# Peiyannn/MM-PDE

Measured on AMD Instinct MI355X. Metric: MM-PDE rollout node-updates/sec, cylinder 2521-node mesh, 1/2/4/8 GPUs, higher is better.
Workload: dtype f32 (every GNN GEMM fp32-emulated by the fp16x3 split with fp32 accumulate: edge message_net_2, node update_net_1/_2 and message_net_1 projections, embedding; DMM, ItpNet, res_cut, kNN and heads exact fp32); 1 GPU; cy-mmpde; trajectories_per_gpu=16, global_trajectories=16, nodes_per_trajectory=2521, neighbors=35, parallelism=trajectory-shard x1 (no data-path collective), rollout=autoregressive (pred -> next input), launch=eager, three HIP streams, stream_priorities=False

## Files before the change

include/mmpde_hip.h:

```cpp
#ifndef MMPDE_HIP_H
#define MMPDE_HIP_H

#include <stdint.h>

#ifdef __cplusplus
extern "C" {
#endif

#define MMPDE_OK 0
#define MMPDE_ERR_INVALID_ARG (-1)
#define MMPDE_ERR_UNSUPPORTED (-2)
#define MMPDE_ERR_HIP_BASE (-1000)

#define MMPDE_ACT_NONE 0
#define MMPDE_ACT_TANH 1
#define MMPDE_ACT_RELU 2
#define MMPDE_ACT_ELU 3
#define MMPDE_PAD_ZEROS 0
#define MMPDE_PAD_CIRCULAR 1

typedef void *mmpde_stream_t;

int mmpde_version(void);
const char *mmpde_status_string(int status);
// ... 43 lines not shown
int mmpde_radius_graph_binned(const float *pos, const void *bins, int64_t batches, int64_t n_per,
                              float r, int max_num_neighbors, int32_t *nbr_out, int32_t *degree_out,
                              int64_t *stats, mmpde_stream_t stream);

int mmpde_edge_index_from_nbr(const int32_t *nbr, int64_t n, int k, int64_t *edge_index,
                              mmpde_stream_t stream);


int mmpde_linear_skinny(const float *x, int64_t ldx, int64_t m, int64_t k, const float *w,
                        int64_t ldw, const float *b, int64_t n, int act, float *y,
                        int64_t ldy, mmpde_stream_t stream);
int64_t mmpde_linear_skinny_workspace_bytes(int64_t m, int64_t n, int64_t k);
int mmpde_linear_skinny_ws(const float *x, int64_t ldx, int64_t m, int64_t k, const float *w,
                           int64_t ldw, const float *b, int64_t n, int act, float *y, int64_t ldy,
                           float *workspace, int64_t workspace_bytes, mmpde_stream_t stream);

int mmpde_traj_mse(const float *pred, const float *labels, int64_t batches, int64_t n_per,
                   float *out, mmpde_stream_t stream);

int mmpde_resample_bilinear(const float *x, int64_t planes, int h, int w, int oh, int ow, float *y,
                            mmpde_stream_t stream);

int mmpde_conv2d(const float *x, int64_t batches, int cin, int h, int w, const float *weight,
                 const float *bias, int cout, int ks, int stride, int pad,
                 const float *residual, int act, float *y, mmpde_stream_t stream);
int mmpde_conv2d_ex(const float *x, int64_t batches, int cin, int h, int w, const float *weight,
                    const float *bias, int cout, int ks, int stride, int pad, int pad_mode,
                    const float *residual, int res_after_act, int act, float *y,
                    mmpde_stream_t stream);

// ... 243 lines not shown
                         const mmpde_dmm_array_branch *br, const mmpde_dmm_head *hd,
                         void *workspace, float *mesh_out, mmpde_stream_t stream);

int64_t mmpde_dmm_head_cache_bytes(int64_t n_per, int hidden);
int mmpde_dmm_head_prepare(const float *xi, int64_t n_per, const mmpde_dmm_head *hd,
                           void *workspace, void *cache, mmpde_stream_t stream);
int mmpde_dmm_mesh_graph_cached(const float *u, const float *grid, int64_t batches,
                                int64_t n_per, const int32_t *grid_nbr, int k,
                                const mmpde_dmm_graph_branch *br, const mmpde_dmm_head *hd,
                                const void *head_cache, void *workspace, float *mesh_out,
                                mmpde_stream_t stream);
int mmpde_dmm_mesh_array_cached(const float *u, const float *xi, int64_t batches, int64_t n_per,
                                const mmpde_dmm_array_branch *br, const mmpde_dmm_head *hd,
                                const void *head_cache, void *workspace, float *mesh_out,
                                mmpde_stream_t stream);

typedef struct {
    const void *head_cache;
    const void *hess_cache;
    float *hess_out;
    float *det_out;
    float *detmin_out;
    int32_t *folds_out;
    int32_t *folds_total;
} mmpde_dmm_hess_io;
int64_t mmpde_dmm_hess_cache_bytes(int64_t n_per, int hidden);
int mmpde_dmm_hess_prepare(const float *xi, int64_t n_per, const mmpde_dmm_head *hd,
                           void *workspace, void *hess_cache, mmpde_stream_t stream);
int64_t mmpde_dmm_hess_workspace_bytes(int64_t batches, int64_t n_per, int latent, int hidden);
int mmpde_dmm_mesh_graph_hess(const float *u, const float *grid, int64_t batches, int64_t n_per,
// ... 60 lines not shown
```

mm-pde_amd/csrc/dense.hip:

```cpp
#include "common.hpp"

namespace {

constexpr int kSkW = 8;
constexpr int kSkMaxZ = 16;

template <int kSkW>
__global__ __launch_bounds__(kSkW * 64) void linear_skinny_kernel(const float *__restrict__ x,
                                                                  int64_t ldx, int64_t m, int64_t k,
                                                                  const float *__restrict__ w,
                                                                  int64_t ldw,
                                                                  const float *__restrict__ b,
                                                                  int64_t n, int act,
                                                                  float *__restrict__ y, int64_t ldy,
                                                                  int nchz, float *__restrict__ part,
                                                                  unsigned *__restrict__ tickets) {
    constexpr int C = 64 * kSkW, LD = C + 4;
    __shared__ float sw[16 * LD], sx[16 * LD];
    const int tid = threadIdx.x;
    const int wave = tid >> 6;
    const int lane = tid & 63;
    const int r = lane & 15, g = lane >> 4;
    const int64_t col0 = (int64_t)blockIdx.x * 16, row0 = (int64_t)blockIdx.y * 16;
    const int K = (int)k;
    const int c0 = (int)blockIdx.z * nchz;
    const int nch = min((K + C - 1) / C - c0, nchz);
    float lw[16], lx[16];
    auto load = [&](int kc) {
        const int kk = kc + tid;
        const bool ok = kk < K;
        const int o = ok ? kk : 0;
#pragma unroll
        for (int i = 0; i < 16; ++i) {
            const float a = w[min(col0 + i, n - 1) * ldw + o];
            const float c = x[min(row0 + i, m - 1) * ldx + o];
            lw[i] = ok ? a : 0.0f;
            lx[i] = ok ? c : 0.0f;
        }
    };
    f32x4 acc = {0.0f, 0.0f, 0.0f, 0.0f};
    if (nch > 0) load(c0 * C);
    for (int c = 0; c < nch; ++c) {
        if (c) __syncthreads();
#pragma unroll
        for (int i = 0; i < 16; ++i) {
            sw[i * LD + tid] = lw[i];
            sx[i * LD + tid] = lx[i];
        }
        __syncthreads();
        if (c + 1 < nch) load((c0 + c + 1) * C);
        const float *aw = sw + r * LD + 64 * wave + 4 * g;
        const float *ax = sx + r * LD + 64 * wave + 4 * g;
#pragma unroll
        for (int q = 0; q < 4; ++q) {
            const float4 wv = *(const float4 *)(aw + 16 * q);
            const float4 xv = *(const float4 *)(ax + 16 * q);
            acc = mfma16(xv.x, wv.x, acc);
            acc = mfma16(xv.y, wv.y, acc);
            acc = mfma16(xv.z, wv.z, acc);
            acc = mfma16(xv.w, wv.w, acc);
        }
    }
    __syncthreads();
    f32x4 *wpart = (f32x4 *)sw;
    wpart[wave * 64 + lane] = acc;
    __syncthreads();
    if (wave != 0) return;
    f32x4 s = wpart[lane];
#pragma unroll
    for (int v = 1; v < kSkW; ++v) s += wpart[v * 64 + lane];
// ... 47 lines not shown
    const float bb = b ? b[col] : 0.0f;
#pragma unroll
    for (int q = 0; q < 4; ++q) {
        const int64_t row = row0 + 4 * g + q;
        if (row < m) y[row * ldy + col] = act_apply(s[q] + bb, act);
    }
}

inline int skinny_splits(int64_t n, int64_t k, int cus) {
    const int64_t ctiles = (n + 15) / 16;
    const int64_t chunks = (k + 64 * kSkW - 1) / (64 * kSkW);
    int64_t z = (4 * (int64_t)cus + ctiles - 1) / ctiles;
    z = z < chunks ? z : chunks;
    z = z < kSkMaxZ ? z : kSkMaxZ;
    return z > 1 ? (int)z : 1;
}

__global__ __launch_bounds__(256) void resample_bilinear_kernel(const float *__restrict__ x, int64_t planes,
                                                                int h, int w, int oh, int ow, float sy,
                                                                float sx, float *__restrict__ y) {
    const int64_t e = (int64_t)blockIdx.x * 256 + threadIdx.x;
    if (e >= planes * oh * ow) return;
    const int ox = (int)(e % ow);
    const int oy = (int)((e / ow) % oh);
    const int64_t pl = e / ((int64_t)ow * oh);
    const float fy = __fmul_rn(sy, (float)oy), fx = __fmul_rn(sx, (float)ox);
    const int y0 = (int)fy, x0 = (int)fx;
    const int y1 = y0 + (y0 < h - 1 ? 1 : 0), x1 = x0 + (x0 < w - 1 ? 1 : 0);
    const float ly = fy - (float)y0, lx = fx - (float)x0;
    const float hy = 1.0f - ly, hx = 1.0f - lx;
// ... 245 lines not shown
        hipDeviceGetAttribute(&cus, hipDeviceAttributeMultiprocessorCount, dev) != hipSuccess || cus < 1)
        return 256;
    return cus;
}

constexpr int64_t kSkTickets = 4096;
static int64_t skinny_ws_bytes(int64_t m, int64_t n, int z) {
    return z > 1 ? (kSkTickets + (int64_t)z * m * n) * (int64_t)sizeof(float) : 0;
}

extern "C" int64_t mmpde_linear_skinny_workspace_bytes(int64_t m, int64_t n, int64_t k) {
    if (m <= 0 || n <= 0 || k <= 0) return 0;
    return skinny_ws_bytes(m, n, skinny_splits(n, k, skinny_cus()));
}

extern "C" int mmpde_linear_skinny_ws(const float *x, int64_t ldx, int64_t m, int64_t k, const float *w,
                                      int64_t ldw, const float *b, int64_t n, int act, float *y, int64_t ldy,
                                      float *workspace, int64_t workspace_bytes, mmpde_stream_t stream) {
    MMPDE_REQUIRE(x && w && y && m > 0 && k > 0 && n > 0 && m <= 4096);
    MMPDE_REQUIRE(ldx >= k && ldw >= k && ldy >= n && act >= 0 && act <= 2);
    hipStream_t st = as_stream(stream);
    int z = skinny_splits(n, k, skinny_cus());
    if (!workspace || workspace_bytes < skinny_ws_bytes(m, n, z)) z = 1;
    const int chunks = ceil_div(k, 64 * kSkW);
    const int nchz = z > 1 ? ceil_div(chunks, z) : chunks;
    z = z > 1 ? ceil_div(chunks, nchz) : 1;
    const int64_t ctiles = ceil_div(n, 16);
    MMPDE_REQUIRE(z == 1 || ctiles <= kSkTickets);
    const int64_t rows_per = z > 1 ? 16 * (kSkTickets / ctiles) : m;
    unsigned *tickets = z > 1 ? (unsigned *)workspace : nullptr;
    float *part = z > 1 ? workspace + kSkTickets : nullptr;
    for (int64_t r0 = 0; r0 < m; r0 += rows_per) {
        const int64_t mr = m - r0 < rows_per ? m - r0 : rows_per;
        const dim3 grid((unsigned)ctiles, (unsigned)ceil_div(mr, 16), (unsigned)z);
        hipLaunchKernelGGL(linear_skinny_kernel<kSkW>, grid, dim3(kSkW * 64), 0, st, x + r0 * ldx, ldx, mr, k, w,
                           ldw, b, n, act, y + r0 * ldy, ldy, nchz, part, tickets);
        MMPDE_RET_LAUNCH();
    }
    return MMPDE_OK;
}

extern "C" int mmpde_linear_skinny(const float *x, int64_t ldx, int64_t m, int64_t k,
                                   const float *w, int64_t ldw, const float *b, int64_t n,
                                   int act, float *y, int64_t ldy, mmpde_stream_t stream) {
    return mmpde_linear_skinny_ws(x, ldx, m, k, w, ldw, b, n, act, y, ldy, nullptr, 0, stream);
}

extern "C" int mmpde_conv2d(const float *x, int64_t batches, int cin, int h, int w,
                            const float *weight, const float *bias, int cout, int ks, int stride,
                            int pad, const float *residual, int act, float *y,
                            mmpde_stream_t stream) {
    MMPDE_REQUIRE(x && weight && y && batches > 0 && cin > 0 && cout > 0 && ks > 0);
    MMPDE_REQUIRE((stride == 1 || stride == 2) && pad >= 0 && act >= 0 && act <= 2);
    const int oh = (h + 2 * pad - ks) / stride + 1;
// ... 74 lines not shown
```

mm-pde_amd/csrc/dmm.hip:

```cpp
#include "common.hpp"
#include "gemm.hpp"

namespace {

struct DmmEmbW {
    float w0[12], b0[4], bn1[16], w3[16], b3[4], bn4[16];
};

__global__ __launch_bounds__(256) void dmm_embed_kernel(const float *__restrict__ u,
                                                        const float2 *__restrict__ grid,
                                                        int64_t n_tot, int64_t n_per,
                                                        mmpde_dmm_graph_branch p,
                                                        float4 *__restrict__ h,
                                                        unsigned *__restrict__ zero, int n_zero) {
    const int64_t i = (int64_t)blockIdx.x * 256 + threadIdx.x;
    if (i < n_zero) zero[i] = 0u;
    if (i >= n_tot) return;
    const float2 g = grid[i % n_per];
    const float in[3] = {u[i], g.x, g.y};
    float z[4], o[4];
#pragma unroll
    for (int c = 0; c < 4; ++c) {
        float v = p.emb0_b[c];
#pragma unroll
// ... 740 lines not shown
    return dmm_head_grid(xi, n_per, hd, w, q, (float2 *)(q + n_per * hd->hidden),
                         as_stream(stream));
}

extern "C" int mmpde_dmm_mesh_graph(const float *u, const float *grid, int64_t batches,
                                    int64_t n_per, const int32_t *grid_nbr, int k,
                                    const mmpde_dmm_graph_branch *br, const mmpde_dmm_head *hd,
                                    void *workspace, float *mesh_out, mmpde_stream_t stream) {
    return mmpde_dmm_mesh_graph_cached(u, grid, batches, n_per, grid_nbr, k, br, hd, nullptr,
                                       workspace, mesh_out, stream);
}

namespace {
int graph_branch(const float *u, const float *grid, int64_t batches, int64_t n_per,
                 const int32_t *grid_nbr, int k, const mmpde_dmm_graph_branch *br, int latent, float *ws,
                 float *sk, int64_t skf, float *branch, float **ws_end, hipStream_t st) {
    const int64_t nt = batches * n_per;
    float4 *h0 = (float4 *)ws;
    float4 *h1 = h0 + nt;
    float *dec = (float *)(h1 + nt);
    float *om1 = dec + ((nt + 3) & ~int64_t(3));
    float *om2 = om1 + batches * 512;
    if (ws_end) *ws_end = om2 + batches * 256;
    const int nz = (int)dmm_skinny_ticket_floats(batches);
    const dim3 g1(ceil_div(nt > nz ? nt : nz, 256)), g4(ceil_div(4 * nt, 256));
    hipLaunchKernelGGL(dmm_embed_kernel, g1, dim3(256), 0, st, u, (const float2 *)grid, nt, n_per,
                       *br, h0, (unsigned *)sk, nz);
    MMPDE_RET_LAUNCH();
    size_t lds = batches <= 65535 ? dmm_gnn_lds_bytes(n_per) : 0;
    if (lds > 64 * 1024 &&
        hipFuncSetAttribute((const void *)dmm_gnn_lds_kernel, hipFuncAttributeMaxDynamicSharedMemorySize,
// ... 10 lines not shown
        } else {
            hipLaunchKernelGGL(dmm_gnn_kernel, g4, dim3(256), 0, st, h0, u, (const float2 *)grid,
                               grid_nbr, k, nt, n_per, br->g_msg1_w[l], br->g_msg1_b[l],
                               br->g_msg2_w[l], br->g_msg2_b[l], br->g_upd1_w[l], br->g_upd1_b[l],
                               br->g_upd2_w[l], br->g_upd2_b[l], br->g_bn_w[l], br->g_bn_b[l],
                               br->g_bn_rm[l], br->g_bn_rv[l], br->eps, h1);
        }
        MMPDE_RET_LAUNCH();
        float4 *t = h0;
        h0 = h1;
        h1 = t;
    }
    hipLaunchKernelGGL(dmm_decode_kernel, g4, dim3(256), 0, st, h0, nt, br->dec0_w, br->dec0_b,
                       br->dec1_w, br->dec1_b, dec);
    MMPDE_RET_LAUNCH();
    int rc = skinny(dec, n_per, batches, n_per, br->om0_w, n_per, br->om0_b, 512, MMPDE_ACT_TANH, om1, 512,
                    sk, skf, st);
    if (rc) return rc;
    rc = skinny(om1, 512, batches, 512, br->om2_w, 512, br->om2_b, 256, MMPDE_ACT_TANH, om2, 256, sk, skf,
                st);
    if (rc) return rc;
    return skinny(om2, 256, batches, 256, br->om4_w, 256, br->om4_b, latent, MMPDE_ACT_NONE, branch, latent,
                  sk, skf, st);
}

int array_branch(const float *u, int64_t batches, const mmpde_dmm_array_branch *br, int latent, float *ws,
                 float *sk, int64_t skf, float *branch, float **ws_end, hipStream_t st) {
    const int s = br->s;
    const int s1 = (s + 4 - 5) / 2 + 1;
    const int s3 = (s1 + 4 - 5) / 2 + 1;
    auto take = [&](int64_t nf) {
        float *p = ws;
// ... 19 lines not shown
    if (rc) return rc;
    rc = skinny(x4, s3 * s3, batches, s3 * s3, br->fc2_w, s3 * s3, br->fc2_b, 1024, MMPDE_ACT_TANH, f2, 1024,
                sk, skf, st);
    if (rc) return rc;
    return skinny(f2, 1024, batches, 1024, br->fc3_w, 1024, br->fc3_b, latent, MMPDE_ACT_NONE, branch, latent,
                  sk, skf, st);
}

int64_t array_n_eff(int64_t n_per, int s) { return n_per > (int64_t)s * s ? n_per : (int64_t)s * s; }
}

namespace {
int mesh_graph(const float *u, const float *grid, int64_t batches, int64_t n_per,
               const int32_t *grid_nbr, int k, const mmpde_dmm_graph_branch *br,
               const mmpde_dmm_head *hd, const void *head_cache, const mmpde_dmm_hess_io *io,
               void *workspace, float *mesh_out, mmpde_stream_t stream) {
    MMPDE_REQUIRE(u && grid && grid_nbr && br && hd && workspace && mesh_out);
    MMPDE_REQUIRE(batches > 0 && n_per > k && k > 0 && br->n_gnn_layers >= 0 &&
                  br->n_gnn_layers <= 3 && al16(workspace));
    if (io && !head_ok(hd)) return MMPDE_ERR_UNSUPPORTED;
    hipStream_t st = as_stream(stream);
    float *ws = (float *)workspace;
    float *sk = ws + dmm_base_floats(batches, n_per, hd->latent, hd->hidden);
    const int64_t skf = dmm_skinny_floats(batches);
    float *end = nullptr;
    const int64_t nt = batches * n_per;
    float *branch = ws + 8 * nt + ((nt + 3) & ~int64_t(3)) + batches * 768;
    float *head_ws = branch + ((batches * hd->latent + 3) & ~int64_t(3));
    int rc = graph_branch(u, grid, batches, n_per, grid_nbr, k, br, hd->latent, ws, sk, skf, branch, &end, st);
    if (rc) return rc;
    if (io) return dmm_head_hess(branch, grid, batches, n_per, hd, head_ws, sk + skf, io, mesh_out, st, sk, skf);
    return dmm_head(branch, grid, batches, n_per, hd, head_ws, (const float *)head_cache, mesh_out,
                    st, sk, skf);
}
}

extern "C" int mmpde_dmm_mesh_graph_cached(const float *u, const float *grid, int64_t batches,
                                           int64_t n_per, const int32_t *grid_nbr, int k,
                                           const mmpde_dmm_graph_branch *br,
                                           const mmpde_dmm_head *hd, const void *head_cache,
                                           void *workspace, float *mesh_out,
                                           mmpde_stream_t stream) {
    return mesh_graph(u, grid, batches, n_per, grid_nbr, k, br, hd, head_cache, nullptr, workspace,
                      mesh_out, stream);
}

extern "C" int mmpde_dmm_mesh_array(const float *u, const float *xi, int64_t batches,
                                    int64_t n_per, const mmpde_dmm_array_branch *br,
                                    const mmpde_dmm_head *hd, void *workspace, float *mesh_out,
                                    mmpde_stream_t stream) {
    return mmpde_dmm_mesh_array_cached(u, xi, batches, n_per, br, hd, nullptr, workspace, mesh_out,
                                       stream);
}

namespace {
int mesh_array(const float *u, const float *xi, int64_t batches, int64_t n_per,
               const mmpde_dmm_array_branch *br, const mmpde_dmm_head *hd, const void *head_cache,
               const mmpde_dmm_hess_io *io, void *workspace, float *mesh_out, mmpde_stream_t stream) {
    MMPDE_REQUIRE(u && xi && br && hd && workspace && mesh_out && batches > 0 && n_per > 0);
// ... 239 lines not shown
```

mm-pde_amd/mmpde_amd/_lib.py:

```python
from __future__ import annotations

import ctypes
import os

import torch

LIB_PATH = os.path.join(os.path.dirname(os.path.abspath(__file__)), "lib", "libmmpde_hip.so")
ABI_VERSION = 12302

ACT_NONE, ACT_TANH, ACT_RELU, ACT_ELU = 0, 1, 2, 3
PAD_ZEROS, PAD_CIRCULAR = 0, 1
EDGE_GEMM = {"f32": 0, "f16x3": 1}

_P = ctypes.c_void_p
_I64 = ctypes.c_int64
_I = ctypes.c_int
_F = ctypes.c_float


class HipExtensionMissing(RuntimeError):
    """libmmpde_hip.so is absent or cannot be loaded (run __graft_entry__.build())."""


class MmpdeError(RuntimeError):
# ... 94 lines not shown
    "mmpde_knn_graph_cand_scratch_bytes": (_I64, [_I64, _I64]),
    "mmpde_knn_skip_threshold": (_I, [_P, _P, _I64, _P, _I, _I, _P, _P]),
    "mmpde_knn_graph_cand": (_I, [_P, _P, _P, _F, _I64, _I64, _I, _P, _P, _P, _P, _P]),
    "mmpde_knn_query_cand": (_I, [_P, _P, _P, _P, _P, _F, _I64, _I64, _I, _P, _P, _P, _P, _P]),
    "mmpde_knn_query": (_I, [_P, _P, _I64, _I64, _I64, _I, _P, _P, _P]),
    "mmpde_knn_bins_grid": (_I, [_I64]),
    "mmpde_knn_bins_bytes": (_I64, [_I64, _I64]),
    "mmpde_knn_bin": (_I, [_P, _I64, _I64, _P, _I64, _P]),
    "mmpde_knn_graph_binned": (_I, [_P, _P, _I64, _I64, _I, _P, _P, _P, _P]),
    "mmpde_knn_query_binned": (_I, [_P, _P, _P, _I64, _I64, _I64, _I, _P, _P, _P, _P]),
    "mmpde_edge_index_from_nbr": (_I, [_P, _I64, _I, _P, _P]),
    "mmpde_linear_skinny": (_I, [_P, _I64, _I64, _I64, _P, _I64, _P, _I64, _I, _P, _I64, _P]),
    "mmpde_linear_skinny_workspace_bytes": (_I64, [_I64, _I64, _I64]),
    "mmpde_linear_skinny_ws": (_I, [_P, _I64, _I64, _I64, _P, _I64, _P, _I64, _I, _P, _I64, _P, _I64,
                                    _P]),
    "mmpde_gnn_edge_backward_ex": (_I, [_P, _P, _P, _P, _I64, _I, _P, _P, _P, _P, _P, _P, _P, _P, _I, _P]),
    "mmpde_traj_mse": (_I, [_P, _P, _I64, _I64, _P, _P]),
    "mmpde_conv2d": (_I, [_P, _I64, _I, _I, _I, _P, _P, _I, _I, _I, _I, _P, _I, _P, _P]),
    "mmpde_resample_bilinear": (_I, [_P, _I64, _I, _I, _I, _I, _P, _P]),
    "mmpde_conv2d_ex": (_I, [_P, _I64, _I, _I, _I, _P, _P, _I, _I, _I, _I, _I, _P, _I, _I, _P, _P]),
    "mmpde_conv2d_grad_weight": (_I, [_P, _I64, _I, _I, _I, _P, _I, _I, _I, _I, _P, _P, _P]),
    "mmpde_rows_grad_weight_workspace_bytes": (_I64, [_I64, _I, _I]),
    "mmpde_reverse_adjacency_scratch_bytes": (_I64, [_I64, _I, _I64]),
    "mmpde_reverse_adjacency": (_I, [_P, _I64, _I, _P, _I64, _P, _P, _P, _P, _I64, _P, _P]),
    "mmpde_gnn_edge_backward_sorted": (_I, [_P, _P, _P, _P, _I64, _I, _P, _P, _P, _P, _P, _P, _P, _P, _P, _P,
                                           _I, _P]),
    "mmpde_gnn_edge_source_sum_sorted": (_I, [_P, _P, _I64, _P, _P]),
    "mmpde_rows_grad_weight": (_I, [_P, _I64, _I64, _I, _P, _I64, _I, _P, _P, _P, _I64, _P]),
    "mmpde_batch_norm_rows_workspace_bytes": (_I64, [_I64, _I]),
    "mmpde_batch_norm_rows_train": (_I, [_P, _P, _I64, _I, _P, _P, _F, _F, _P, _P, _P, _P, _P, _I64, _P]),
# ... 119 lines not shown
```

mm-pde_amd/mmpde_amd/dmm_model.py:

```python
from __future__ import annotations

import ctypes

import torch
from torch import nn

from . import _lib as L
from .gnn_2d import BatchNorm
from . import ops
from .ops import knn_graph_nbr




class DenseNet(nn.Module):

    def __init__(self, layers, width=32, normalize=False):
        super().__init__()
        if normalize:
            raise NotImplementedError("DenseNet(normalize=True) is not used by MM-PDE")
        self.n_layers = len(layers) - 1
        assert self.n_layers >= 1
        self.layers = nn.ModuleList(nn.Linear(a, b) for a, b in zip(layers[:-1], layers[1:]))
        self.normalize = normalize
# ... 89 lines not shown
            self.embedding_mlp = nn.Sequential(
                nn.Linear(3, self.hidden_features), nn.BatchNorm1d(self.hidden_features),
                nn.Tanh(), nn.Linear(self.hidden_features, self.hidden_features),
                nn.BatchNorm1d(self.hidden_features))
            self.decoding_mlp = DenseNet([self.hidden_features, 128, 1])
            self.output_mlp = nn.Sequential(
                nn.Linear(grid.shape[0], 512), nn.Tanh(), nn.Linear(512, 256), nn.Tanh(),
                nn.Linear(256, trunk_layer[-1]))
            self.trunk = DenseNet(trunk_layer)
            self.out_nn = DenseNet(out_layer)
        else:
            raise ValueError(mode)
        self._pack_key = None
        self._pack = None
        self._grid_cache = {}

    def forward(self, u, grid, rf=False):
        L.require_device(u, grid)
        if self.training:
            return self._forward_train(u, grid, rf)
        bp, hd = self.device_params()
        u = L.f32c(u)
        grid = L.f32c(grid).reshape(-1, 2)
        B, ng = u.shape[0], grid.shape[0]
        if ng % B:
            raise ValueError("grid rows must be a multiple of the batch size")
        lib = L.lib()
        st = L.stream(u.device)
        branch = self.branch_features(u)
        nb = lib.mmpde_dmm_phi_workspace_bytes(B, ng, hd.latent, hd.hidden, hd.th)
# ... 183 lines not shown
        B, N = u.shape[0], xi.shape[0]
        if workspace is None:
            ne = N if self.mode == "graph" else max(N, self.branch.s ** 2)
            nb = L.lib().mmpde_dmm_workspace_bytes(B, ne, hd.latent, hd.hidden)
            workspace = torch.empty((nb // 4,), dtype=torch.float32, device=u.device)
        if out is None:
            out = torch.empty((B * N, 2), dtype=torch.float32, device=u.device)
        if head_cache is not None:
            L.require_device(head_cache)
            if head_cache.numel() * 4 < L.lib().mmpde_dmm_head_cache_bytes(N, hd.hidden):
                raise ValueError("head_cache is smaller than mmpde_dmm_head_cache_bytes")
        hc = L.ptr(head_cache) if head_cache is not None else None
        st = L.stream(u.device)
        if self.mode == "graph":
            nbr = self.grid_nbr(xi) if nbr is None else self._local_nbr(nbr, N, u.device)
            L.check(L.lib().mmpde_dmm_mesh_graph_cached(
                L.ptr(u), L.ptr(xi), B, N, L.ptr(nbr), nbr.shape[1], ctypes.byref(bp),
                ctypes.byref(hd), hc, L.ptr(workspace), L.ptr(out), st), "mmpde_dmm_mesh_graph")
        else:
            if nbr is not None:
                raise ValueError("nbr is a graph-mode argument")
            L.check(L.lib().mmpde_dmm_mesh_array_cached(
                L.ptr(u), L.ptr(xi), B, N, ctypes.byref(bp), ctypes.byref(hd), hc,
                L.ptr(workspace), L.ptr(out), st), "mmpde_dmm_mesh_array")
        return out

    def hess_cache(self, xi: torch.Tensor, workspace: torch.Tensor | None = None) -> torch.Tensor:
        L.require_device(xi)
        _, hd = self.device_params()
        xi = L.f32c(xi).reshape(-1, 2)
# ... 109 lines not shown
```

mm-pde_amd/mmpde_amd/interpolate.py:

```python
from __future__ import annotations

import ctypes

import torch
from torch import nn

from . import _lib as L
from . import ops


def _mlp(widths):
    return nn.ModuleList(nn.Linear(a, b) for a, b in zip(widths[:-1], widths[1:]))


class ResCutMlp(torch.autograd.Function):

    @staticmethod
    def forward(ctx, x, *params):
        ws, bs = params[0::2], params[1::2]
        acts = (L.ACT_TANH, L.ACT_TANH, L.ACT_TANH, L.ACT_NONE)
        ins = [L.f32c(x)]
        for w, b, act in zip(ws, bs, acts):
            ins.append(ops.linear_skinny(ins[-1], w, b, act))
        y = ins.pop()
# ... 51 lines not shown
        self.n_layers3 = len(self.layers3_node) - 1
        self.layers3 = _mlp(self.layers3_node)
        self.conv = ori_ny is not None
        if self.conv:
            c = layers3
            self.down = nn.Sequential(
                nn.Conv2d(c[0], c[1], 5, padding=2), nn.Tanh(),
                nn.Conv2d(c[1], c[2], 5, padding=2), nn.Tanh(),
                nn.Conv2d(c[2], c[3], 5, padding=2), nn.Tanh(),
                nn.Conv2d(c[3], c[4], 5, padding=2), nn.Tanh())
        else:
            self.down = nn.Sequential(
                nn.Linear(ori_nx, 2048), nn.Tanh(), nn.Linear(2048, 512), nn.Tanh(),
                nn.Linear(512, 2048), nn.Tanh(), nn.Linear(2048, ori_nx))
        self._packs = {}

    def packed(self, mode: str) -> torch.Tensor:
        mods = self.layers if mode == "1" else self.layers2
        if [m.out_features for m in mods] != [128, 64, 30] or mods[0].in_features != 62:
            raise NotImplementedError("fused ItpNet kernel needs layers [62, 128, 64, 30] "
                                      "(the reference defaults --itpnet_node1/2 = 128,64)")
        ts = [t for m in mods for t in (m.weight, m.bias)]
        key = tuple((t.data_ptr(), t._version) for t in ts)
        hit = self._packs.get(mode)
        if hit is not None and hit[0] == key:
            return hit[1]
        L.require_device(*ts)
        f = [L.f32c(t) for t in ts]
        mlp = L.ItpMlp(*[t.data_ptr() for t in f])
        buf = torch.empty((L.lib().mmpde_itp_pack_bytes() // 4,), dtype=torch.float32,
# ... 30 lines not shown
            if self.conv:
                x = data
                for i in (0, 2, 4, 6):
                    x = torch.tanh(ops.Conv2dSame.apply(x, d[i].weight, d[i].bias, False))
                return x
            params = [t for i in (0, 2, 4, 6) for t in (d[i].weight, d[i].bias)]
            return ResCutMlp.apply(data.reshape(data.shape[0], -1), *params)
        if self.conv:
            x = data
            for i in (0, 2, 4, 6):
                x = ops.conv2d(x, d[i].weight, d[i].bias, 1, 2, L.ACT_TANH)
            return x
        x = data.reshape(data.shape[0], -1)
        layers = [(d[i].weight, d[i].bias, act)
                  for i, act in ((0, L.ACT_TANH), (2, L.ACT_TANH), (4, L.ACT_TANH), (6, L.ACT_NONE))]
        for w, b, act in layers:
            x = ops.linear_skinny(x, w, b, act)
        return x

    def forward(self, neighbors, query_points, mode, data=None):
        if mode == "res_cut":
            return self.res_cut(data)
        if mode in ("1", "2"):
            return self.weights(neighbors, query_points, mode)
        return data
```

mm-pde_amd/mmpde_amd/ops.py:

```python
from __future__ import annotations

import ctypes

import os

import torch

from . import _lib as L
from . import rows

KNN_MAX_POINTS = 65536
KNN_TILE_POINTS = 4096


def _knn_points_check(n_per: int, k: int, what: str):
    if n_per > KNN_MAX_POINTS:
        raise ValueError(f"{what}: {n_per} points per trajectory; the HIP kNN kernels take at "
                         f"most {KNN_MAX_POINTS} (run --base_resolution <= 256 x 256)")
    if k > 63:
        raise ValueError(f"{what}: k = {k}; the HIP kNN kernels take k <= 63")


KNN_BINNED_MIN_POINTS = 4097
KNN_METHODS = ("full", "binned")
# ... 166 lines not shown
    def mode(self, role) -> str:
        return self.state[role]["mode"]

    def after_table(self, role, cells: torch.Tensor, column: int) -> None:
        st = self.state[role]
        st["since"] += 1
        if st["pending"] is not None or (st["mode"] == "table" and (st["since"] - 1) % self.CHECK_EVERY):
            return
        if _capturing():
            if st["mode"] == "probe":
                st["mode"], st["wait"] = "full", self.PROBE_EVERY
            return
        miss = torch.empty((self.B, 2), dtype=torch.int32, device=self.device)
        L.check(L.lib().mmpde_knn_table_misses(L.ptr(cells), self.B, L.ptr(miss), L.stream(self.device)),
                "mmpde_knn_table_misses")
        host = torch.empty((self.B,), dtype=torch.int32, pin_memory=True)
        host.copy_(miss[:, column], non_blocking=True)
        ev = torch.cuda.Event()
        ev.record()
        st["pending"] = (ev, host)


def _cand_scratch(scratch, batches, N, device):
    need = L.lib().mmpde_knn_graph_cand_scratch_bytes(batches, N)
    if scratch is None or scratch.numel() * scratch.element_size() < need:
        scratch = torch.empty((max(need, 1),), dtype=torch.uint8, device=device)
    return scratch


def knn_graph_moved(pos: torch.Tensor, xi: torch.Tensor, cand, batches: int, k: int,
                    scratch: torch.Tensor | None = None, count_degenerate: bool = False,
                    cells: torch.Tensor | None = None, skip_above: float = 0.0):
    if cand is None:
        return knn_graph_nbr(pos, batches, k, count_degenerate)
    L.require_device(pos)
# ... 163 lines not shown
    return idx


_SKINNY_WS = {}


def _skinny_workspace(device, nbytes: int) -> torch.Tensor:
    key = (str(device), torch.cuda.current_stream(device).cuda_stream)
    ws = _SKINNY_WS.get(key)
    if ws is None or ws.numel() * 4 < nbytes:
        ws = torch.zeros((max(nbytes, 4) // 4 + 1024,), dtype=torch.float32, device=device)
        _SKINNY_WS[key] = ws
    return ws


def linear_skinny(x: torch.Tensor, w: torch.Tensor, b=None, act: int = L.ACT_NONE,
                  out: torch.Tensor | None = None) -> torch.Tensor:
    L.require_device(x, w)
    x = L.f32c(x)
    w = L.f32c(w)
    m, k = x.shape
    n = w.shape[0]
    y = out if out is not None else torch.empty((m, n), dtype=torch.float32, device=x.device)
    lib = L.lib()
    wsb = lib.mmpde_linear_skinny_workspace_bytes(m, n, k)
    ws = _skinny_workspace(x.device, wsb)
    L.check(lib.mmpde_linear_skinny_ws(L.ptr(x), k, m, k, L.ptr(w), k,
                                       L.ptr(L.f32c(b)) if b is not None else None, n, act,
                                       L.ptr(y), n, L.ptr(ws), wsb, L.stream(x.device)),
            "mmpde_linear_skinny")
    return y


def linear_rows(x: torch.Tensor, w: torch.Tensor, b=None, act: int = L.ACT_NONE) -> torch.Tensor:
    lead = x.shape[:-1]
    x2 = L.f32c(x).reshape(-1, x.shape[-1])
    y = torch.empty((x2.shape[0], w.shape[0]), dtype=torch.float32, device=x2.device)
    for r0 in range(0, x2.shape[0], 4096):
        linear_skinny(x2[r0:r0 + 4096], w, b, act, out=y[r0:r0 + 4096])
    return y.reshape(*lead, w.shape[0])


def resample_bilinear(u: torch.Tensor, oh: int, ow: int) -> torch.Tensor:
# ... 351 lines not shown
```

Before: 21.53 million node-updates/s.

## Pre-pack large skinny-GEMM weights into per-lane MFMA fragment layout

Adds a packing kernel that rearranges large weight matrices into a tile-major image matching the per-lane float4 fragments the skinny MFMA kernel consumes. A PACKED kernel variant loads weight fragments straight from global memory into registers, skipping the LDS staging and strided per-row loads. Packs are cached per weight (keyed by pointer and version) and used for the DMM output_mlp[0] and the interpolation down-projection layers when the weight has more than 2^20 elements. A minor tweak also copies the full miss table to host and slices it afterwards. The cost is extra memory for the packed images and a repack whenever a weight changes.

New measurement: 21.58 million node-updates/s, median of 6. Within noise of the previous version (+0.2%).

```diff
diff --git a/include/mmpde_hip.h b/include/mmpde_hip.h
--- a/include/mmpde_hip.h
+++ b/include/mmpde_hip.h
@@ -81,6 +81,13 @@
 int mmpde_linear_skinny_ws(const float *x, int64_t ldx, int64_t m, int64_t k, const float *w,
                            int64_t ldw, const float *b, int64_t n, int act, float *y, int64_t ldy,
                            float *workspace, int64_t workspace_bytes, mmpde_stream_t stream);
+int64_t mmpde_linear_skinny_pack_bytes(int64_t n, int64_t k);
+int mmpde_linear_skinny_pack(const float *w, int64_t ldw, int64_t n, int64_t k, float *image,
+                             mmpde_stream_t stream);
+int mmpde_linear_skinny_packed_ws(const float *x, int64_t ldx, int64_t m, int64_t k,
+                                  const float *image, int64_t image_bytes, const float *b, int64_t n,
+                                  int act, float *y, int64_t ldy, float *workspace,
+                                  int64_t workspace_bytes, mmpde_stream_t stream);
 
 int mmpde_traj_mse(const float *pred, const float *labels, int64_t batches, int64_t n_per,
                    float *out, mmpde_stream_t stream);
@@ -354,6 +361,12 @@
                                 const mmpde_dmm_array_branch *br, const mmpde_dmm_head *hd,
                                 const void *head_cache, void *workspace, float *mesh_out,
                                 mmpde_stream_t stream);
+int mmpde_dmm_mesh_graph_packed(const float *u, const float *grid, int64_t batches,
+                                int64_t n_per, const int32_t *grid_nbr, int k,
+                                const mmpde_dmm_graph_branch *br, const mmpde_dmm_head *hd,
+                                const void *head_cache, const float *om0_image,
+                                int64_t om0_image_bytes, void *workspace, float *mesh_out,
+                                mmpde_stream_t stream);
 
 typedef struct {
     const void *head_cache;
diff --git a/mm-pde_amd/csrc/dense.hip b/mm-pde_amd/csrc/dense.hip
--- a/mm-pde_amd/csrc/dense.hip
+++ b/mm-pde_amd/csrc/dense.hip
@@ -5,7 +5,7 @@
 constexpr int kSkW = 8;
 constexpr int kSkMaxZ = 16;
 
-template <int kSkW>
+template <int kSkW, bool PACKED>
 __global__ __launch_bounds__(kSkW * 64) void linear_skinny_kernel(const float *__restrict__ x,
                                                                   int64_t ldx, int64_t m, int64_t k,
                                                                   const float *__restrict__ w,
@@ -16,7 +16,7 @@
                                                                   int nchz, float *__restrict__ part,
                                                                   unsigned *__restrict__ tickets) {
     constexpr int C = 64 * kSkW, LD = C + 4;
-    __shared__ float sw[16 * LD], sx[16 * LD];
+    __shared__ __align__(16) float sw[PACKED ? 4 * 64 * kSkW : 16 * LD], sx[16 * LD];
     const int tid = threadIdx.x;
     const int wave = tid >> 6;
     const int lane = tid & 63;
@@ -25,16 +25,27 @@
     const int K = (int)k;
     const int c0 = (int)blockIdx.z * nchz;
     const int nch = min((K + C - 1) / C - c0, nchz);
-    float lw[16], lx[16];
+    float lw[PACKED ? 1 : 16], lx[16];
+    float4 pw[4];
+    const float4 *img = nullptr;
+    if (PACKED)
+        img = (const float4 *)w + (int64_t)blockIdx.x * ((K + C - 1) / C) * (4 * C) + wave * 256 + lane;
     auto load = [&](int kc) {
         const int kk = kc + tid;
         const bool ok = kk < K;
         const int o = ok ? kk : 0;
+        if (PACKED) {
+            const float4 *p = img + (int64_t)(kc / C) * (4 * C);
+#pragma unroll
+            for (int q = 0; q < 4; ++q) pw[q] = p[64 * q];
+        }
 #pragma unroll
         for (int i = 0; i < 16; ++i) {
-            const float a = w[min(col0 + i, n - 1) * ldw + o];
+            if (!PACKED) {
+                const float a = w[min(col0 + i, n - 1) * ldw + o];
+                lw[i] = ok ? a : 0.0f;
+            }
             const float c = x[min(row0 + i, m - 1) * ldx + o];
-            lw[i] = ok ? a : 0.0f;
             lx[i] = ok ? c : 0.0f;
         }
     };
@@ -44,16 +55,17 @@
         if (c) __syncthreads();
 #pragma unroll
         for (int i = 0; i < 16; ++i) {
-            sw[i * LD + tid] = lw[i];
+            if (!PACKED) sw[i * LD + tid] = lw[i];
             sx[i * LD + tid] = lx[i];
         }
+        const float4 cw[4] = {pw[0], pw[1], pw[2], pw[3]};
         __syncthreads();
         if (c + 1 < nch) load((c0 + c + 1) * C);
-        const float *aw = sw + r * LD + 64 * wave + 4 * g;
+        const float *aw = PACKED ? sw : sw + r * LD + 64 * wave + 4 * g;
         const float *ax = sx + r * LD + 64 * wave + 4 * g;
 #pragma unroll
         for (int q = 0; q < 4; ++q) {
-            const float4 wv = *(const float4 *)(aw + 16 * q);
+            const float4 wv = PACKED ? cw[q] : *(const float4 *)(aw + 16 * q);
             const float4 xv = *(const float4 *)(ax + 16 * q);
             acc = mfma16(xv.x, wv.x, acc);
             acc = mfma16(xv.y, wv.y, acc);
@@ -131,6 +143,28 @@
     z = z < chunks ? z : chunks;
     z = z < kSkMaxZ ? z : kSkMaxZ;
     return z > 1 ? (int)z : 1;
+}
+
+constexpr int kSkBlock = 16 * 64 * kSkW;
+inline int64_t skinny_pack_floats(int64_t n, int64_t k) {
+    return ((n + 15) / 16) * ((k + 64 * kSkW - 1) / (64 * kSkW)) * kSkBlock;
+}
+__global__ __launch_bounds__(256) void skinny_pack_kernel(const float *__restrict__ w, int64_t ldw, int64_t n,
+                                                          int64_t k, int64_t chunks, int64_t total4,
+                                                          float4 *__restrict__ img) {
+    const int64_t e = (int64_t)blockIdx.x * 256 + threadIdx.x;
+    if (e >= total4) return;
+    const int lane = (int)(e & 63), q = (int)(e >> 6) & 3, wave = (int)((e >> 8) % kSkW);
+    const int64_t blk = e / (kSkBlock / 4);
+    const int64_t row = (blk / chunks) * 16 + (lane & 15);
+    const int64_t kk = (blk % chunks) * (64 * kSkW) + 64 * wave + 16 * q + 4 * (lane >> 4);
+    const float *p = w + row * ldw + kk;
+    float4 v;
+    v.x = row < n && kk < k ? p[0] : 0.0f;
+    v.y = row < n && kk + 1 < k ? p[1] : 0.0f;
+    v.z = row < n && kk + 2 < k ? p[2] : 0.0f;
+    v.w = row < n && kk + 3 < k ? p[3] : 0.0f;
+    img[e] = v;
 }
 
 __global__ __launch_bounds__(256) void resample_bilinear_kernel(const float *__restrict__ x, int64_t planes,
@@ -406,9 +440,25 @@
     return skinny_ws_bytes(m, n, skinny_splits(n, k, skinny_cus()));
 }
 
-extern "C" int mmpde_linear_skinny_ws(const float *x, int64_t ldx, int64_t m, int64_t k, const float *w,
-                                      int64_t ldw, const float *b, int64_t n, int act, float *y, int64_t ldy,
-                                      float *workspace, int64_t workspace_bytes, mmpde_stream_t stream) {
+extern "C" int64_t mmpde_linear_skinny_pack_bytes(int64_t n, int64_t k) {
+    if (n <= 0 || k <= 0) return 0;
+    return skinny_pack_floats(n, k) * (int64_t)sizeof(float);
+}
+
+extern "C" int mmpde_linear_skinny_pack(const float *w, int64_t ldw, int64_t n, int64_t k, float *image,
+                                        mmpde_stream_t stream) {
+    MMPDE_REQUIRE(w && image && n > 0 && k > 0 && ldw >= k && k < ((int64_t)1 << 31));
+    MMPDE_REQUIRE(((uintptr_t)image & 15u) == 0);
+    const int64_t total4 = skinny_pack_floats(n, k) / 4;
+    hipLaunchKernelGGL(skinny_pack_kernel, dim3((unsigned)ceil_div(total4, 256)), dim3(256), 0, as_stream(stream),
+                       w, ldw, n, k, (int64_t)ceil_div(k, 64 * kSkW), total4, (float4 *)image);
+    MMPDE_RET_LAUNCH();
+    return MMPDE_OK;
+}
+
+static int skinny_launch(const float *x, int64_t ldx, int64_t m, int64_t k, const float *w, int64_t ldw,
+                         bool packed, const float *b, int64_t n, int act, float *y, int64_t ldy,
+                         float *workspace, int64_t workspace_bytes, mmpde_stream_t stream) {
     MMPDE_REQUIRE(x && w && y && m > 0 && k > 0 && n > 0 && m <= 4096);
     MMPDE_REQUIRE(ldx >= k && ldw >= k && ldy >= n && act >= 0 && act <= 2);
     hipStream_t st = as_stream(stream);
@@ -425,11 +475,30 @@
     for (int64_t r0 = 0; r0 < m; r0 += rows_per) {
         const int64_t mr = m - r0 < rows_per ? m - r0 : rows_per;
         const dim3 grid((unsigned)ctiles, (unsigned)ceil_div(mr, 16), (unsigned)z);
-        hipLaunchKernelGGL(linear_skinny_kernel<kSkW>, grid, dim3(kSkW * 64), 0, st, x + r0 * ldx, ldx, mr, k, w,
-                           ldw, b, n, act, y + r0 * ldy, ldy, nchz, part, tickets);
+        if (packed)
+            hipLaunchKernelGGL((linear_skinny_kernel<kSkW, true>), grid, dim3(kSkW * 64), 0, st, x + r0 * ldx, ldx,
+                               mr, k, w, ldw, b, n, act, y + r0 * ldy, ldy, nchz, part, tickets);
+        else
+            hipLaunchKernelGGL((linear_skinny_kernel<kSkW, false>), grid, dim3(kSkW * 64), 0, st, x + r0 * ldx, ldx,
+                               mr, k, w, ldw, b, n, act, y + r0 * ldy, ldy, nchz, part, tickets);
         MMPDE_RET_LAUNCH();
     }
     return MMPDE_OK;
+}
+
+extern "C" int mmpde_linear_skinny_ws(const float *x, int64_t ldx, int64_t m, int64_t k, const float *w,
+                                      int64_t ldw, const float *b, int64_t n, int act, float *y, int64_t ldy,
+                                      float *workspace, int64_t workspace_bytes, mmpde_stream_t stream) {
+    return skinny_launch(x, ldx, m, k, w, ldw, false, b, n, act, y, ldy, workspace, workspace_bytes, stream);
+}
+
+extern "C" int mmpde_linear_skinny_packed_ws(const float *x, int64_t ldx, int64_t m, int64_t k,
+                                             const float *image, int64_t image_bytes, const float *b, int64_t n,
+                                             int act, float *y, int64_t ldy, float *workspace,
+                                             int64_t workspace_bytes, mmpde_stream_t stream) {
+    MMPDE_REQUIRE(image && ((uintptr_t)image & 15u) == 0 && n > 0 && k > 0);
+    MMPDE_REQUIRE(image_bytes >= mmpde_linear_skinny_pack_bytes(n, k));
+    return skinny_launch(x, ldx, m, k, image, k, true, b, n, act, y, ldy, workspace, workspace_bytes, stream);
 }
 
 extern "C" int mmpde_linear_skinny(const float *x, int64_t ldx, int64_t m, int64_t k,
diff --git a/mm-pde_amd/csrc/dmm.hip b/mm-pde_amd/csrc/dmm.hip
--- a/mm-pde_amd/csrc/dmm.hip
+++ b/mm-pde_amd/csrc/dmm.hip
@@ -778,7 +778,8 @@
 namespace {
 int graph_branch(const float *u, const float *grid, int64_t batches, int64_t n_per,
                  const int32_t *grid_nbr, int k, const mmpde_dmm_graph_branch *br, int latent, float *ws,
-                 float *sk, int64_t skf, float *branch, float **ws_end, hipStream_t st) {
+                 float *sk, int64_t skf, float *branch, float **ws_end, hipStream_t st,
+                 const float *om0_img = nullptr, int64_t om0_bytes = 0) {
     const int64_t nt = batches * n_per;
     float4 *h0 = (float4 *)ws;
     float4 *h1 = h0 + nt;
@@ -819,8 +820,11 @@
     hipLaunchKernelGGL(dmm_decode_kernel, g4, dim3(256), 0, st, h0, nt, br->dec0_w, br->dec0_b,
                        br->dec1_w, br->dec1_b, dec);
     MMPDE_RET_LAUNCH();
-    int rc = skinny(dec, n_per, batches, n_per, br->om0_w, n_per, br->om0_b, 512, MMPDE_ACT_TANH, om1, 512,
-                    sk, skf, st);
+    int rc = om0_img ? mmpde_linear_skinny_packed_ws(dec, n_per, batches, n_per, om0_img, om0_bytes, br->om0_b,
+                                                     512, MMPDE_ACT_TANH, om1, 512, sk,
+                                                     skf * (int64_t)sizeof(float), st)
+                     : skinny(dec, n_per, batches, n_per, br->om0_w, n_per, br->om0_b, 512, MMPDE_ACT_TANH, om1,
+                              512, sk, skf, st);
     if (rc) return rc;
     rc = skinny(om1, 512, batches, 512, br->om2_w, 512, br->om2_b, 256, MMPDE_ACT_TANH, om2, 256, sk, skf,
                 st);
@@ -870,7 +874,8 @@
 int mesh_graph(const float *u, const float *grid, int64_t batches, int64_t n_per,
                const int32_t *grid_nbr, int k, const mmpde_dmm_graph_branch *br,
                const mmpde_dmm_head *hd, const void *head_cache, const mmpde_dmm_hess_io *io,
-               void *workspace, float *mesh_out, mmpde_stream_t stream) {
+               void *workspace, float *mesh_out, mmpde_stream_t stream, const float *om0_img = nullptr,
+               int64_t om0_bytes = 0) {
     MMPDE_REQUIRE(u && grid && grid_nbr && br && hd && workspace && mesh_out);
     MMPDE_REQUIRE(batches > 0 && n_per > k && k > 0 && br->n_gnn_layers >= 0 &&
                   br->n_gnn_layers <= 3 && al16(workspace));
@@ -883,7 +888,8 @@
     const int64_t nt = batches * n_per;
     float *branch = ws + 8 * nt + ((nt + 3) & ~int64_t(3)) + batches * 768;
     float *head_ws = branch + ((batches * hd->latent + 3) & ~int64_t(3));
-    int rc = graph_branch(u, grid, batches, n_per, grid_nbr, k, br, hd->latent, ws, sk, skf, branch, &end, st);
+    int rc = graph_branch(u, grid, batches, n_per, grid_nbr, k, br, hd->latent, ws, sk, skf, branch, &end, st,
+                          om0_img, om0_bytes);
     if (rc) return rc;
     if (io) return dmm_head_hess(branch, grid, batches, n_per, hd, head_ws, sk + skf, io, mesh_out, st, sk, skf);
     return dmm_head(branch, grid, batches, n_per, hd, head_ws, (const float *)head_cache, mesh_out,
@@ -899,6 +905,17 @@
                                            mmpde_stream_t stream) {
     return mesh_graph(u, grid, batches, n_per, grid_nbr, k, br, hd, head_cache, nullptr, workspace,
                       mesh_out, stream);
+}
+
+extern "C" int mmpde_dmm_mesh_graph_packed(const float *u, const float *grid, int64_t batches,
+                                           int64_t n_per, const int32_t *grid_nbr, int k,
+                                           const mmpde_dmm_graph_branch *br,
+                                           const mmpde_dmm_head *hd, const void *head_cache,
+                                           const float *om0_image, int64_t om0_image_bytes,
+                                           void *workspace, float *mesh_out, mmpde_stream_t stream) {
+    MMPDE_REQUIRE(om0_image);
+    return mesh_graph(u, grid, batches, n_per, grid_nbr, k, br, hd, head_cache, nullptr, workspace,
+                      mesh_out, stream, om0_image, om0_image_bytes);
 }
 
 extern "C" int mmpde_dmm_mesh_array(const float *u, const float *xi, int64_t batches,
diff --git a/mm-pde_amd/mmpde_amd/_lib.py b/mm-pde_amd/mmpde_amd/_lib.py
--- a/mm-pde_amd/mmpde_amd/_lib.py
+++ b/mm-pde_amd/mmpde_amd/_lib.py
@@ -132,6 +132,11 @@
     "mmpde_linear_skinny_workspace_bytes": (_I64, [_I64, _I64, _I64]),
     "mmpde_linear_skinny_ws": (_I, [_P, _I64, _I64, _I64, _P, _I64, _P, _I64, _I, _P, _I64, _P, _I64,
                                     _P]),
+    "mmpde_linear_skinny_pack_bytes": (_I64, [_I64, _I64]),
+    "mmpde_linear_skinny_pack": (_I, [_P, _I64, _I64, _I64, _P, _P]),
+    "mmpde_linear_skinny_packed_ws": (_I, [_P, _I64, _I64, _I64, _P, _I64, _P, _I64, _I, _P, _I64, _P, _I64,
+                                           _P]),
+    "mmpde_dmm_mesh_graph_packed": (_I, [_P, _P, _I64, _I64, _P, _I, _P, _P, _P, _P, _I64, _P, _P, _P]),
     "mmpde_gnn_edge_backward_ex": (_I, [_P, _P, _P, _P, _I64, _I, _P, _P, _P, _P, _P, _P, _P, _P, _I, _P]),
     "mmpde_traj_mse": (_I, [_P, _P, _I64, _I64, _P, _P]),
     "mmpde_conv2d": (_I, [_P, _I64, _I, _I, _I, _P, _P, _I, _I, _I, _I, _P, _I, _P, _P]),
diff --git a/mm-pde_amd/mmpde_amd/dmm_model.py b/mm-pde_amd/mmpde_amd/dmm_model.py
--- a/mm-pde_amd/mmpde_amd/dmm_model.py
+++ b/mm-pde_amd/mmpde_amd/dmm_model.py
@@ -127,6 +127,7 @@
         self._pack_key = None
         self._pack = None
         self._grid_cache = {}
+        self._skinny_packs = ops.SkinnyPacks()
 
     def forward(self, u, grid, rf=False):
         L.require_device(u, grid)
@@ -340,6 +341,14 @@
         st = L.stream(u.device)
         if self.mode == "graph":
             nbr = self.grid_nbr(xi) if nbr is None else self._local_nbr(nbr, N, u.device)
+            om0 = self.output_mlp[0].weight
+            if ops.SKINNY_PACKED and om0.numel() >= ops.SKINNY_PACK_MIN_WEIGHTS:
+                img = self._skinny_packs.get("output_mlp.0", om0)
+                L.check(L.lib().mmpde_dmm_mesh_graph_packed(
+                    L.ptr(u), L.ptr(xi), B, N, L.ptr(nbr), nbr.shape[1], ctypes.byref(bp),
+                    ctypes.byref(hd), hc, L.ptr(img), img.numel() * 4, L.ptr(workspace), L.ptr(out), st),
+                    "mmpde_dmm_mesh_graph_packed")
+                return out
             L.check(L.lib().mmpde_dmm_mesh_graph_cached(
                 L.ptr(u), L.ptr(xi), B, N, L.ptr(nbr), nbr.shape[1], ctypes.byref(bp),
                 ctypes.byref(hd), hc, L.ptr(workspace), L.ptr(out), st), "mmpde_dmm_mesh_graph")
diff --git a/mm-pde_amd/mmpde_amd/interpolate.py b/mm-pde_amd/mmpde_amd/interpolate.py
--- a/mm-pde_amd/mmpde_amd/interpolate.py
+++ b/mm-pde_amd/mmpde_amd/interpolate.py
@@ -89,6 +89,7 @@
                 nn.Linear(ori_nx, 2048), nn.Tanh(), nn.Linear(2048, 512), nn.Tanh(),
                 nn.Linear(512, 2048), nn.Tanh(), nn.Linear(2048, ori_nx))
         self._packs = {}
+        self._skinny_packs = ops.SkinnyPacks()
 
     def packed(self, mode: str) -> torch.Tensor:
         mods = self.layers if mode == "1" else self.layers2
@@ -149,9 +150,14 @@
         x = data.reshape(data.shape[0], -1)
         layers = [(d[i].weight, d[i].bias, act)
                   for i, act in ((0, L.ACT_TANH), (2, L.ACT_TANH), (4, L.ACT_TANH), (6, L.ACT_NONE))]
-        for w, b, act in layers:
-            x = ops.linear_skinny(x, w, b, act)
+        for i, (w, b, act) in enumerate(layers):
+            x = ops.linear_skinny(x, w, b, act, pack=self.down_pack(i, w))
         return x
+
+    def down_pack(self, i: int, w: torch.Tensor):
+        if not ops.SKINNY_PACKED or w.numel() < ops.SKINNY_PACK_MIN_WEIGHTS:
+            return None
+        return self._skinny_packs.get(f"down.{i}", w)
 
     def forward(self, neighbors, query_points, mode, data=None):
         if mode == "res_cut":
diff --git a/mm-pde_amd/mmpde_amd/ops.py b/mm-pde_amd/mmpde_amd/ops.py
--- a/mm-pde_amd/mmpde_amd/ops.py
+++ b/mm-pde_amd/mmpde_amd/ops.py
@@ -204,11 +204,11 @@
         miss = torch.empty((self.B, 2), dtype=torch.int32, device=self.device)
         L.check(L.lib().mmpde_knn_table_misses(L.ptr(cells), self.B, L.ptr(miss), L.stream(self.device)),
                 "mmpde_knn_table_misses")
-        host = torch.empty((self.B,), dtype=torch.int32, pin_memory=True)
-        host.copy_(miss[:, column], non_blocking=True)
+        host = torch.empty((self.B, 2), dtype=torch.int32, pin_memory=True)
+        host.copy_(miss, non_blocking=True)
         ev = torch.cuda.Event()
         ev.record()
-        st["pending"] = (ev, host)
+        st["pending"] = (ev, host[:, column])
 
 
 def _cand_scratch(scratch, batches, N, device):
@@ -402,19 +402,64 @@
     return ws
 
 
+SKINNY_PACKED = True
+SKINNY_PACK_MIN_WEIGHTS = (1 << 20) + 1
+
+
+def skinny_pack_index(n: int, k: int):
+    import numpy as np
+
+    tiles, chunks = (n + 15) // 16, (k + 511) // 512
+    e = np.arange(tiles * chunks * 8192, dtype=np.int64)
+    t, lane, q, wave, blk = e & 3, (e >> 2) & 63, (e >> 8) & 3, (e >> 10) & 7, e >> 13
+    row = (blk // chunks) * 16 + (lane & 15)
+    col = (blk % chunks) * 512 + 64 * wave + 16 * q + 4 * (lane >> 4) + t
+    return row, col
+
+
+def skinny_pack(w: torch.Tensor) -> torch.Tensor:
+    L.require_device(w)
+    w = L.f32c(w)
+    n, k = w.shape
+    img = torch.empty((L.lib().mmpde_linear_skinny_pack_bytes(n, k) // 4,), dtype=torch.float32,
+                      device=w.device)
+    L.check(L.lib().mmpde_linear_skinny_pack(L.ptr(w), k, n, k, L.ptr(img), L.stream(w.device)),
+            "mmpde_linear_skinny_pack")
+    return img
+
+
+class SkinnyPacks:
+
+    def __init__(self):
+        self._hit = {}
+
+    def get(self, name: str, w: torch.Tensor) -> torch.Tensor:
+        key = (w.data_ptr(), w._version, tuple(w.shape))
+        hit = self._hit.get(name)
+        if hit is None or hit[0] != key:
+            hit = self._hit[name] = (key, skinny_pack(w))
+        return hit[1]
+
+
 def linear_skinny(x: torch.Tensor, w: torch.Tensor, b=None, act: int = L.ACT_NONE,
-                  out: torch.Tensor | None = None) -> torch.Tensor:
-    L.require_device(x, w)
+                  out: torch.Tensor | None = None, pack: torch.Tensor | None = None) -> torch.Tensor:
+    L.require_device(x, w, pack)
     x = L.f32c(x)
-    w = L.f32c(w)
     m, k = x.shape
     n = w.shape[0]
     y = out if out is not None else torch.empty((m, n), dtype=torch.float32, device=x.device)
     lib = L.lib()
     wsb = lib.mmpde_linear_skinny_workspace_bytes(m, n, k)
     ws = _skinny_workspace(x.device, wsb)
-    L.check(lib.mmpde_linear_skinny_ws(L.ptr(x), k, m, k, L.ptr(w), k,
-                                       L.ptr(L.f32c(b)) if b is not None else None, n, act,
+    bf = L.f32c(b) if b is not None else None
+    bp = L.ptr(bf)
+    if pack is not None:
+        L.check(lib.mmpde_linear_skinny_packed_ws(L.ptr(x), k, m, k, L.ptr(pack), pack.numel() * 4, bp, n,
+                                                  act, L.ptr(y), n, L.ptr(ws), wsb, L.stream(x.device)),
+                "mmpde_linear_skinny_packed")
+        return y
+    w = L.f32c(w)
+    L.check(lib.mmpde_linear_skinny_ws(L.ptr(x), k, m, k, L.ptr(w), k, bp, n, act,
                                        L.ptr(y), n, L.ptr(ws), wsb, L.stream(x.device)),
             "mmpde_linear_skinny")
     return y
```
